# SandAI-org/MagiAttention

Measured on AMD Instinct MI355X. Metric: attention TFLOPS/sec fwd+bwd (whole-job; per-GPU = value/n_gpus); cp scaling at seqlen 64k, higher is better.
Workload: dtype bf16; 1 GPU; dense_causal_64k_h32_d128; seqlen=65536, heads=32, kv_heads=32, head_dim=128, mask=causal, global_batch=1, parallelism=cp1

## Files before the change

### magi_attention/csrc/ffa_bwd.hip

```cpp

#include <hip/hip_runtime.h>
#include <math.h>
#include <stdlib.h>

#include "../../include/magi_ffa.h"
#include "ffa_device.h"

#define BWD_BN 32
#define BWD_BM 32

DEV_INLINE bool wave_alive(int m0, int qe) { return m0 < qe; }

struct BwdParams {
  const bf16_t* dout;
  const bf16_t* q;
  const bf16_t* k;
  const bf16_t* v;
  const void* out;
  const float* lse;
  float* dq;
  float* dk;
  float* dv;
  float* dpsum;
  const int* q_ranges;
  const int* k_ranges;
  const int* attn_type_map;
  int hq, hk, gqa;
  float scale;
  float softcap;
  long long total_q, total_k;
  int head_major;
  int work_nx, work_ny, work_nz;
  int head_mult;
  int head_off;
  int n_heads_launch;
  const int* seg_starts;
};

template <bool OUT_F32>
__global__ __launch_bounds__(256) void bwd_preprocess_kernel(BwdParams p, int d,
                                                             long long n_rows) {
  const long long row = (long long)blockIdx.x * 4 + (threadIdx.x >> 6);
  if (row >= n_rows) return;
  const int lane = threadIdx.x & 63;
  const int per = d / 64;
  const bf16_t* do_p = p.dout + row * d;
  float acc = 0.f;
  for (int e = 0; e < per; ++e) {
    const int idx = lane * per + e;
    const float dov = (float)do_p[idx];
    float ov;
    if (OUT_F32)
      ov = ((const float*)p.out)[row * d + idx];
    else
      ov = (float)((const bf16_t*)p.out)[row * d + idx];
    acc += dov * ov;
  }
#pragma unroll
  for (int s = 32; s > 0; s >>= 1) acc += __shfl_xor(acc, s, 64);
  if (lane == 0) p.dpsum[row] = acc;
}


template <int D, bool HAS_SOFTCAP, int MODE, int WAVES>
__global__ __launch_bounds__(64 * WAVES, WAVES == 8 ? 2 : 1)
void ffa_bwd_dkv_kernel(BwdParams p) {
  static_assert(WAVES == 4 || (WAVES == 8 && D != 192), "unsupported shape");
  constexpr int NBUF = (MODE != 0 && WAVES == 8) ? 3 : 2;
  constexpr bool WANT_DV = MODE != 2;
  constexpr bool WANT_DK = MODE != 1;
  constexpr bool V_IN_LDS = MODE == 0;
  constexpr int DF = D / 16;
  constexpr int DT = D / 32;
  constexpr int ROWB = (D == 192) ? 512 : D * 2;
  constexpr int ROWE = ROWB / 2;
  constexpr int VSLOTS = D / 8;
  constexpr int SW32M = ROWB / 32 - 1;
  auto swz = [](int row, int byte_off) {
    return byte_off ^ ((row & SW32M) << 5);
  };
  const long long work_total =
      (long long)p.work_nx * p.work_ny * p.work_nz;
  const long long grid_span = (long long)gridDim.x * gridDim.y * gridDim.z;
  const long long w_first = blockIdx.x +
      (long long)gridDim.x * (blockIdx.y + (long long)gridDim.y * blockIdx.z);
  for (long long w = w_first; w < work_total; w += grid_span) {
  const int wx = (int)(w % p.work_nx);
  const long long w2 = w / p.work_nx;
  const int wy = (int)(w2 % p.work_ny);
  const int wz = (int)(w2 / p.work_ny);
  const int ri = wz;
  const int hidx = p.head_major ? wx : wy;
  const int h = p.head_off + hidx * p.head_mult;
  const int wb = p.head_major ? wy : wx;
  const int ks = p.k_ranges[2 * ri], ke = p.k_ranges[2 * ri + 1];
  const int nblk0 = ks + wb * (BWD_BN * WAVES);
  if (nblk0 >= ke) continue;
  const int seg0 = p.seg_starts ? p.seg_starts[ri] : ri;
  const int seg1 = p.seg_starts ? p.seg_starts[ri + 1] : ri + 1;
  int qs, qe, atype;

  const int tid = threadIdx.x;
  const int lane = tid & 63;
  const int wave = tid >> 6;
  if (WAVES == 8 && wave >= 4) asm volatile("s_setprio 1");

  const int lo32 = lane & 31;
  const int hi = lane >> 5;

  const int n0 = nblk0 + wave * BWD_BN;
  const bool wave_live = n0 < ke;

  const float sl2 = HAS_SOFTCAP ? p.softcap * 1.4426950408889634f
                                : p.scale * 1.4426950408889634f;
  const float cap_pre = HAS_SOFTCAP ? p.scale / p.softcap : 0.f;
  const float log2e = 1.4426950408889634f;

  const int kh = h / p.gqa;
  const size_t k_pitch = (size_t)p.hk * D;
  const size_t q_pitch = (size_t)p.hq * D;

  constexpr int QITER =
      (V_IN_LDS && D == 128 && WAVES == 8) ? BWD_BM : 2 * BWD_BM;
  constexpr int NSUB = QITER / BWD_BM;
  constexpr int KVLDS = V_IN_LDS ? 2 * WAVES * BWD_BN * ROWB : 0;
  constexpr int LSELDS = V_IN_LDS ? 0 : NBUF * 2 * QITER * 4;
  static_assert(NBUF * 2 * QITER * ROWB + LSELDS + KVLDS <= 163840,
                "LDS budget");
  __shared__ __attribute__((aligned(16))) char smem[
      NBUF * 2 * QITER * ROWB + LSELDS + KVLDS];
  auto lds_q = [&](int buf) -> __bf16* {
    return (__bf16*)(smem + (2 * buf) * QITER * ROWB);
  };
  auto lds_do = [&](int buf) -> __bf16* {
    return (__bf16*)(smem + (2 * buf + 1) * QITER * ROWB);
  };
  auto lds_lse = [&](int buf) -> float* {
    return (float*)(smem + NBUF * 2 * QITER * ROWB + buf * 2 * QITER * 4);
  };
  __bf16* lds_kt = (__bf16*)(smem + NBUF * 2 * QITER * ROWB + LSELDS) +
                   wave * BWD_BN * ROWE;
  __bf16* lds_vt = (__bf16*)(smem + NBUF * 2 * QITER * ROWB + LSELDS +
                             KVLDS / 2) +
                   wave * BWD_BN * ROWE;

  const int krow = n0 + lo32;
  const int kcl = min(krow, ke - 1);
  const bf16_t* kp_row = p.k + (size_t)kcl * k_pitch + (size_t)kh * D + hi * 8;
  bf16x8 kfA[V_IN_LDS ? 1 : DF], vfA[(WANT_DK && !V_IN_LDS) ? DF : 1];
  if constexpr (!V_IN_LDS) {
    const bf16_t* vp = p.v + (size_t)kcl * k_pitch + (size_t)kh * D;
#pragma unroll
    for (int dd = 0; dd < DF; ++dd) {
      kfA[dd] = *(const bf16x8*)(kp_row - hi * 8 + dd * 16 + hi * 8);
      if constexpr (WANT_DK)
        vfA[dd] = *(const bf16x8*)(vp + dd * 16 + hi * 8);
    }
  }
  constexpr int ROWS_PER_GLDS_V = 1024 / ROWB;
  if constexpr (V_IN_LDS) {
#pragma unroll
    for (int gi = 0; gi < BWD_BN / ROWS_PER_GLDS_V; ++gi) {
      const int r0v = ROWS_PER_GLDS_V * gi;
      const int r = r0v + lane / (ROWB / 16);
      const int c = lane % (ROWB / 16);
      const int kr = min(n0 + r, ke - 1);
      int cs = c ^ ((r & SW32M) << 1);
      if (cs >= VSLOTS) cs = 0;
      const int csw = cs * 8;
      __builtin_amdgcn_global_load_lds(
          (const __attribute__((address_space(1))) unsigned int*)(
              p.k + (size_t)kr * k_pitch + (size_t)kh * D + csw),
          (__attribute__((address_space(3))) unsigned int*)&lds_kt[r0v * ROWE],
          16, 0, 0);
      __builtin_amdgcn_global_load_lds(
          (const __attribute__((address_space(1))) unsigned int*)(
              p.v + (size_t)kr * k_pitch + (size_t)kh * D + csw),
          (__attribute__((address_space(3))) unsigned int*)&lds_vt[r0v * ROWE],
          16, 0, 0);
    }
  }

  const int nlast = min(nblk0 + BWD_BN * WAVES, ke) - 1;
  int q_lo = 0, q_hi = 0, wq_lo = 0, wq_hi = 0;
  auto seg_bounds = [&]() {
    q_lo = qs; q_hi = qe;
    if (atype == 1 || atype == 3) q_lo = max(q_lo, nblk0 - (ke - qe));
    if (atype == 2 || atype == 3) q_hi = min(q_hi, nlast - (ks - qs) + 1);
    wq_lo = qs; wq_hi = qe;
    if (atype == 1 || atype == 3) wq_lo = max(wq_lo, n0 - (ke - qe));
    if (atype == 2 || atype == 3)
      wq_hi = min(wq_hi, (n0 + BWD_BN - 1) - (ks - qs) + 1);
  };

  f32x16 acc_dk[WANT_DK ? DT : 1], acc_dv[WANT_DV ? DT : 1];
#pragma unroll
  for (int dt = 0; dt < DT; ++dt) {
    if constexpr (WANT_DK) acc_dk[dt] = (f32x16)(0.f);
    if constexpr (WANT_DV) acc_dv[dt] = (f32x16)(0.f);
  }

  constexpr int ROWS_PER_GLDS = 1024 / ROWB;
  constexpr int GLDS_TOTAL = QITER / ROWS_PER_GLDS;
  static_assert(NBUF == 2 || GLDS_TOTAL % WAVES == 0, "uniform stage count");
  constexpr int GLDS_PER_WAVE =
      (GLDS_TOTAL % WAVES == 0) ? GLDS_TOTAL / WAVES : 0;
  auto stage_glds = [&](int buf, int m0x) {
#pragma unroll
    for (int gi0 = 0; gi0 < (GLDS_TOTAL + WAVES - 1) / WAVES; ++gi0) {
      const int gi = gi0 * WAVES + wave;
      if (GLDS_TOTAL % WAVES != 0 && gi >= GLDS_TOTAL) break;
      const int r0 = ROWS_PER_GLDS * gi;
      const int r = r0 + lane / (ROWB / 16);
      const int c = lane % (ROWB / 16);
      const int qrow = min(m0x + r, qe - 1);
      int cs = c ^ ((r & SW32M) << 1);
      if (cs >= VSLOTS) cs = 0;
      const int csw = cs * 8;
      __builtin_amdgcn_global_load_lds(
          (const __attribute__((address_space(1))) unsigned int*)(
              p.q + (size_t)qrow * q_pitch + (size_t)h * D + csw),
          (__attribute__((address_space(3))) unsigned int*)&lds_q(buf)[r0 * ROWE],
          16, 0, 0);
      __builtin_amdgcn_global_load_lds(
          (const __attribute__((address_space(1))) unsigned int*)(
              p.dout + (size_t)qrow * q_pitch + (size_t)h * D + csw),
          (__attribute__((address_space(3))) unsigned int*)&lds_do(buf)[r0 * ROWE],
          16, 0, 0);
    }
    if constexpr (!V_IN_LDS) {
#pragma unroll
      for (int sg = 0; sg < NSUB; ++sg) {
        const int qr = min(m0x + sg * BWD_BM + lo32, qe - 1);
        const float* src = (lane < 32) ? p.lse + (size_t)qr * p.hq + h
                                       : p.dpsum + (size_t)qr * p.hq + h;
        __builtin_amdgcn_global_load_lds(
            (const __attribute__((address_space(1))) unsigned int*)src,
            (__attribute__((address_space(3))) unsigned int*)(
                lds_lse(buf) + sg * 2 * BWD_BM),
            4, 0, 0);
      }
    }
  };

  constexpr int GOPS = 2 * GLDS_PER_WAVE + 2;
  int cur = 0;
  for (int seg = seg0; seg < seg1; ++seg) {
  qs = p.q_ranges[2 * seg];
  qe = p.q_ranges[2 * seg + 1];
  atype = p.attn_type_map ? p.attn_type_map[seg] : 0;
  if (qe <= qs) continue;
  seg_bounds();
  if (q_lo >= q_hi) continue;
  cur = 0;
  stage_glds(0, q_lo);
  if constexpr (NBUF == 3) stage_glds(1, q_lo + QITER);

  for (int m0 = q_lo; m0 < q_hi; m0 += QITER) {
    pipe_barrier<NBUF == 3 ? GOPS : 0>();
    if constexpr (NBUF == 3) {
      stage_glds(cur == 0 ? 2 : cur - 1, m0 + 2 * QITER);
    } else {
      if (m0 + QITER < q_hi) stage_glds(cur ^ 1, m0 + QITER);
    }
#pragma unroll
    for (int sub = 0; sub < NSUB; ++sub) {
    const int ms = m0 + sub * BWD_BM;
    if (ms >= q_hi) break;
    const __bf16* lqb = lds_q(cur) + sub * BWD_BM * ROWE;
    const __bf16* ldb = lds_do(cur) + sub * BWD_BM * ROWE;
    const float* lse_t = nullptr;
    const float* dps_t = nullptr;
    float lsedp_reg = 0.f;
    if constexpr (!V_IN_LDS) {
      lse_t = lds_lse(cur) + sub * 2 * BWD_BM;
      dps_t = lse_t + BWD_BM;
    } else {
      const int qr = min(ms + lo32, qe - 1);
      lsedp_reg = (lane < 32) ? p.lse[(size_t)qr * p.hq + h]
                              : p.dpsum[(size_t)qr * p.hq + h];
    }
    auto lse_at = [&](int rl) -> float {
      if constexpr (!V_IN_LDS) return lse_t[rl];
      return __uint_as_float(__builtin_amdgcn_ds_bpermute(
          rl << 2, __float_as_uint(lsedp_reg)));
    };
    auto dps_at = [&](int rl) -> float {
      if constexpr (!V_IN_LDS) return dps_t[rl];
      return __uint_as_float(__builtin_amdgcn_ds_bpermute(
          (32 + rl) << 2, __float_as_uint(lsedp_reg)));
    };

    if (wave_live && ms + BWD_BM > wq_lo && ms < wq_hi) {
      f32x16 s = (f32x16)(0.f), dp = (f32x16)(0.f);
      if constexpr (V_IN_LDS) {
        const char* kt_c = (const char*)lds_kt;
        const char* vt_c = (const char*)lds_vt;
#pragma unroll
        for (int dd = 0; dd < DF; ++dd) {
          const int off = swz(lo32, lo32 * ROWB + dd * 32 + hi * 16);
          bf16x8 dof = *(const bf16x8*)((const char*)ldb + off);
          bf16x8 vf = *(const bf16x8*)(vt_c + off);
          dp = __builtin_amdgcn_mfma_f32_32x32x16_bf16(dof, vf, dp, 0, 0, 0);
          bf16x8 qf = *(const bf16x8*)((const char*)lqb + off);
          bf16x8 kf = *(const bf16x8*)(kt_c + off);
          s = __builtin_amdgcn_mfma_f32_32x32x16_bf16(qf, kf, s, 0, 0, 0);
        }
      } else {
#pragma unroll
      for (int dd = 0; dd < DF; ++dd) {
        const int off = swz(lo32, lo32 * ROWB + dd * 32 + hi * 16);
        bf16x8 qf = *(const bf16x8*)((const char*)lqb + off);
        s = __builtin_amdgcn_mfma_f32_32x32x16_bf16(qf, kfA[dd], s, 0, 0, 0);
        if constexpr (WANT_DK) {
          bf16x8 dof = *(const bf16x8*)((const char*)ldb + off);
          dp = __builtin_amdgcn_mfma_f32_32x32x16_bf16(dof, vfA[dd], dp, 0, 0, 0);
        }
      }
      }

      const int kk = n0 + lo32;
      float* pv = (float*)&s;
      float* dsv = (float*)&dp;
      const bool interior =
          (ms + BWD_BM <= wq_hi) && (ms >= qs) && (n0 + BWD_BN <= ke) &&
          !((atype == 1 || atype == 3) && (n0 + BWD_BN - 1 > ms + (ke - qe))) &&
          !((atype == 2 || atype == 3) && (n0 < ms + BWD_BM - 1 + (ks - qs)));
      bool all_live = interior;
      if (interior) {
#pragma unroll
        for (int r = 0; r < 16; ++r) {
          const float lq = lse_at(crow(r, hi));
          all_live = all_live && (lq != INFINITY) && (lq != -INFINITY);
        }
      }
      if (__all(all_live) && !HAS_SOFTCAP) {
#pragma unroll
        for (int r = 0; r < 16; ++r) {
          const int rl = crow(r, hi);
          const float pij = fast_exp2(s[r] * sl2 - lse_at(rl) * log2e);
          if constexpr (WANT_DV) pv[r] = pij;
          if constexpr (WANT_DK)
            dsv[r] = pij * (dp[r] - dps_at(rl)) * p.scale;
        }
      } else {
#pragma unroll
        for (int r = 0; r < 16; ++r) {
          const int qrow = ms + crow(r, hi);
          const float lq = (qrow < qe) ? lse_at(crow(r, hi)) : INFINITY;
          bool ok = (qrow < wq_hi) && (qrow >= qs) && lq != INFINITY &&
                    lq != -INFINITY && kk < ke;
          if (atype == 1 || atype == 3) ok = ok && (kk - qrow <= ke - qe);
          if (atype == 2 || atype == 3) ok = ok && (kk - qrow >= ks - qs);
          float sv = s[r];
          float dscale = p.scale;
          float t;
          if (HAS_SOFTCAP) {
            const float th = tanhf(sv * cap_pre);
            t = th * sl2;
            dscale = p.scale * (1.f - th * th);
          } else {
            t = sv * sl2;
          }
          const float pij = ok ? fast_exp2(t - lq * log2e) : 0.f;
          if constexpr (WANT_DV) pv[r] = pij;
          if constexpr (WANT_DK)
            dsv[r] = pij * (dp[r] - dps_at(crow(r, hi))) * dscale;
        }
      }

      {
        const int qhalf = (lane >> 4) & 1;
        const int jrow = (lane & 15) >> 2;
        const int row0 = 8 * hi + jrow;
        const int row1 = 8 * hi + 4 + jrow;
        const int q_base = (int)(unsigned long long)(
            (__attribute__((address_space(3))) const char*)lqb);
        const int do_base = (int)(unsigned long long)(
            (__attribute__((address_space(3))) const char*)ldb);
        const int lane8 = (lane & 3) * 8;
        const int sw0 = (row0 & SW32M) << 5;
        const int sw1 = (row1 & SW32M) << 5;
        const int rb0 = row0 * ROWB + lane8;
        const int rb1 = row1 * ROWB + lane8;
        const int sw2 = ((row0 + 16) & SW32M) << 5;
        const int sw3 = ((row1 + 16) & SW32M) << 5;
        const int rb2 = (row0 + 16) * ROWB + lane8;
        const int rb3 = (row1 + 16) * ROWB + lane8;
        auto pipe_mm = [&](int tbase, bf16x8 a0, bf16x8 a1, f32x16* acc) {
          bf16x8 bcur = tr16_frag(tbase + rb0 + ((16 * qhalf * 2) ^ sw0),
                                  tbase + rb1 + ((16 * qhalf * 2) ^ sw1));
#pragma unroll
          for (int j = 0; j < 2 * DT; ++j) {
            bf16x8 bnext = bcur;
            if (j + 1 < 2 * DT) {
              const int dcoln = (((j + 1) >> 1) * 32 + 16 * qhalf) * 2;
              if ((j + 1) & 1)
                bnext = tr16_frag(tbase + rb2 + (dcoln ^ sw2),
                                  tbase + rb3 + (dcoln ^ sw3));
              else
                bnext = tr16_frag(tbase + rb0 + (dcoln ^ sw0),
                                  tbase + rb1 + (dcoln ^ sw1));
            }
            acc[j >> 1] = __builtin_amdgcn_mfma_f32_32x32x16_bf16(
                (j & 1) ? a1 : a0, bcur, acc[j >> 1], 0, 0, 0);
            bcur = bnext;
          }
        };
        if constexpr (MODE == 1) {
          pipe_mm(do_base, cframe_to_afrag(pv, 0), cframe_to_afrag(pv, 1),
                  acc_dv);
        } else if constexpr (MODE == 2) {
          pipe_mm(q_base, cframe_to_afrag(dsv, 0), cframe_to_afrag(dsv, 1),
                  acc_dk);
        } else {
          bf16x8 pa0 = cframe_to_afrag(pv, 0);
          bf16x8 pa1 = cframe_to_afrag(pv, 1);
          bf16x8 da0 = cframe_to_afrag(dsv, 0);
          bf16x8 da1 = cframe_to_afrag(dsv, 1);
#pragma unroll
          for (int dt = 0; dt < DT; ++dt) {
            const int dcol = (dt * 32 + 16 * qhalf) * 2;
            bf16x8 bdo = tr16_frag(do_base + rb0 + (dcol ^ sw0),
                                   do_base + rb1 + (dcol ^ sw1));
            acc_dv[dt] = __builtin_amdgcn_mfma_f32_32x32x16_bf16(
                pa0, bdo, acc_dv[dt], 0, 0, 0);
            bf16x8 bq = tr16_frag(q_base + rb0 + (dcol ^ sw0),
                                  q_base + rb1 + (dcol ^ sw1));
            acc_dk[dt] = __builtin_amdgcn_mfma_f32_32x32x16_bf16(
                da0, bq, acc_dk[dt], 0, 0, 0);
            bf16x8 bdo1 = tr16_frag(do_base + rb2 + (dcol ^ sw2),
                                    do_base + rb3 + (dcol ^ sw3));
            acc_dv[dt] = __builtin_amdgcn_mfma_f32_32x32x16_bf16(
                pa1, bdo1, acc_dv[dt], 0, 0, 0);
            bf16x8 bq1 = tr16_frag(q_base + rb2 + (dcol ^ sw2),
                                   q_base + rb3 + (dcol ^ sw3));
            acc_dk[dt] = __builtin_amdgcn_mfma_f32_32x32x16_bf16(
                da1, bq1, acc_dk[dt], 0, 0, 0);
          }
        }
      }
    }
    }
    cur = (NBUF == 3) ? (cur == 2 ? 0 : cur + 1) : (cur ^ 1);
  }
  __syncthreads();
  }

  if (wave_live) {
#pragma unroll
  for (int r = 0; r < 16; ++r) {
    const int kr = n0 + crow(r, hi);
    if (kr >= ke) continue;
    float* dkp = p.dk + (size_t)kr * k_pitch + (size_t)kh * D;
    float* dvp = p.dv + (size_t)kr * k_pitch + (size_t)kh * D;
#pragma unroll
    for (int dt = 0; dt < DT; ++dt) {
      if constexpr (WANT_DK) {
        if (acc_dk[dt][r] != 0.f)
          unsafeAtomicAdd(dkp + dt * 32 + lo32, acc_dk[dt][r]);
      }
      if constexpr (WANT_DV) {
        if (acc_dv[dt][r] != 0.f)
          unsafeAtomicAdd(dvp + dt * 32 + lo32, acc_dv[dt][r]);
      }
    }
  }
  }
  if constexpr (MODE == 0) break;
  }
}


template <int D, bool HAS_SOFTCAP, int WAVES>
__global__ __launch_bounds__(64 * WAVES, WAVES == 8 ? 1 : 2)
void ffa_bwd_dq_kernel(BwdParams p) {
  static_assert(WAVES == 4 || (WAVES == 8 && D != 192), "unsupported shape");
  constexpr int NBUF = WAVES == 8 ? 3 : 2;
  constexpr int DF = D / 16;
  constexpr int DT = D / 32;
  constexpr int ROWB = (D == 192) ? 512 : D * 2;
  constexpr int ROWE = ROWB / 2;
  constexpr int VSLOTS = D / 8;
  constexpr int SW32M = ROWB / 32 - 1;
  auto swz = [](int row, int byte_off) {
    return byte_off ^ ((row & SW32M) << 5);
  };
  const long long work_total =
      (long long)p.work_nx * p.work_ny * p.work_nz;
  const long long grid_span = (long long)gridDim.x * gridDim.y * gridDim.z;
  for (long long w = blockIdx.x +
           (long long)gridDim.x * (blockIdx.y + (long long)gridDim.y * blockIdx.z);
       w < work_total; w += grid_span) {
  const int wx = (int)(w % p.work_nx);
  const long long w2 = w / p.work_nx;
  const int wy = (int)(w2 % p.work_ny);
  const int wz = (int)(w2 / p.work_ny);
  const int ri = wz;
  const int h = p.head_major ? wx : wy;
  const int wb = p.head_major ? wy : wx;
  const int qs = p.q_ranges[2 * ri], qe = p.q_ranges[2 * ri + 1];
  const int mblk0 = qs + wb * (BWD_BM * WAVES);
  if (mblk0 >= qe) continue;
  const int seg0 = p.seg_starts ? p.seg_starts[ri] : ri;
  const int seg1 = p.seg_starts ? p.seg_starts[ri + 1] : ri + 1;
  int ks, ke, atype;

  const int tid = threadIdx.x;
  const int lane = tid & 63;
  const int wave = tid >> 6;
  if (WAVES == 8 && wave >= 4) asm volatile("s_setprio 1");

  const int lo32 = lane & 31;
  const int hi = lane >> 5;

  const int m0 = mblk0 + wave * BWD_BM;
  const int qrow = m0 + lo32;
  const bool qvalid = qrow < qe && m0 < qe;
  const int qcl = qvalid ? qrow : (qe - 1);

  const float sl2 = HAS_SOFTCAP ? p.softcap * 1.4426950408889634f
                                : p.scale * 1.4426950408889634f;
  const float cap_pre = HAS_SOFTCAP ? p.scale / p.softcap : 0.f;
  const float log2e = 1.4426950408889634f;

  const int kh = h / p.gqa;
  const size_t k_pitch = (size_t)p.hk * D;
  const size_t q_pitch = (size_t)p.hq * D;

  constexpr int KITER = 2 * BWD_BN;
  static_assert(NBUF * 2 * KITER * ROWB <= 163840, "LDS budget");
  __shared__ __attribute__((aligned(16))) char smem[NBUF * 2 * KITER * ROWB];
  auto lds_k = [&](int buf) -> __bf16* {
    return (__bf16*)(smem + (2 * buf) * KITER * ROWB);
  };
  auto lds_v = [&](int buf) -> __bf16* {
    return (__bf16*)(smem + (2 * buf + 1) * KITER * ROWB);
  };

  bf16x8 qf[DF], dof[DF];
  {
    const bf16_t* qp = p.q + (size_t)qcl * q_pitch + (size_t)h * D;
    const bf16_t* dp = p.dout + (size_t)qcl * q_pitch + (size_t)h * D;
#pragma unroll
    for (int dd = 0; dd < DF; ++dd) {
      qf[dd] = *(const bf16x8*)(qp + dd * 16 + hi * 8);
      dof[dd] = *(const bf16x8*)(dp + dd * 16 + hi * 8);
    }
  }
  const float lse_q = qvalid ? p.lse[(size_t)qrow * p.hq + h] : INFINITY;
  const float dpsum_q = qvalid ? p.dpsum[(size_t)qrow * p.hq + h] : 0.f;
  const bool row_live = qvalid && lse_q != INFINITY && lse_q != -INFINITY;

  const int mlast = min(mblk0 + BWD_BM * WAVES, qe) - 1;
  int k_lo = 0, k_hi = 0, wk_lo = 0, wk_hi = 0;
  auto seg_bounds = [&]() {
    k_lo = ks; k_hi = ke;
    if (atype == 1 || atype == 3) k_hi = min(k_hi, mlast + (ke - qe) + 1);
    if (atype == 2 || atype == 3) k_lo = max(k_lo, mblk0 + (ks - qs));
    wk_lo = ks; wk_hi = ke;
    if (atype == 1 || atype == 3)
      wk_hi = min(wk_hi, min(m0 + BWD_BM, qe) - 1 + (ke - qe) + 1);
    if (atype == 2 || atype == 3) wk_lo = max(wk_lo, m0 + (ks - qs));
  };

  f32x16 acc_dq[DT];
#pragma unroll
  for (int dt = 0; dt < DT; ++dt) acc_dq[dt] = (f32x16)(0.f);

  constexpr int ROWS_PER_GLDS = 1024 / ROWB;
  static_assert(KITER / WAVES >= ROWS_PER_GLDS, "stage rows per wave");
  constexpr int GLDS_PER_WAVE = (KITER / WAVES) / ROWS_PER_GLDS;
  auto stage_glds = [&](int buf, int n0x) {
#pragma unroll
    for (int gi = 0; gi < GLDS_PER_WAVE; ++gi) {
      const int r0 = (KITER / WAVES) * wave + ROWS_PER_GLDS * gi;
      const int r = r0 + lane / (ROWB / 16);
      const int c = lane % (ROWB / 16);
      const int kr = min(n0x + r, ke - 1);
      int cs = c ^ ((r & SW32M) << 1);
      if (cs >= VSLOTS) cs = 0;
      const int csw = cs * 8;
      __builtin_amdgcn_global_load_lds(
          (const __attribute__((address_space(1))) unsigned int*)(
              p.k + (size_t)kr * k_pitch + (size_t)kh * D + csw),
          (__attribute__((address_space(3))) unsigned int*)&lds_k(buf)[r0 * ROWE],
          16, 0, 0);
      __builtin_amdgcn_global_load_lds(
          (const __attribute__((address_space(1))) unsigned int*)(
              p.v + (size_t)kr * k_pitch + (size_t)kh * D + csw),
          (__attribute__((address_space(3))) unsigned int*)&lds_v(buf)[r0 * ROWE],
          16, 0, 0);
    }
  };

  constexpr int GOPS = 2 * GLDS_PER_WAVE;
  int cur = 0;
  for (int seg = seg0; seg < seg1; ++seg) {
  ks = p.k_ranges[2 * seg];
  ke = p.k_ranges[2 * seg + 1];
  atype = p.attn_type_map ? p.attn_type_map[seg] : 0;
  if (ke <= ks) continue;
  seg_bounds();
  if (k_lo >= k_hi) continue;
  cur = 0;
  stage_glds(0, k_lo);
  if constexpr (NBUF == 3) stage_glds(1, k_lo + KITER);

  for (int n0 = k_lo; n0 < k_hi; n0 += KITER) {
    pipe_barrier<NBUF == 3 ? GOPS : 0>();
    if constexpr (NBUF == 3) {
      stage_glds(cur == 0 ? 2 : cur - 1, n0 + 2 * KITER);
    } else {
      if (n0 + KITER < k_hi) stage_glds(cur ^ 1, n0 + KITER);
    }
#pragma unroll
    for (int sub = 0; sub < 2; ++sub) {
    const int ns = n0 + sub * BWD_BN;
    if (ns >= k_hi) break;
    const __bf16* lkb = lds_k(cur) + sub * BWD_BN * ROWE;
    const __bf16* lvb = lds_v(cur) + sub * BWD_BN * ROWE;

    if (wave_alive(m0, qe) && ns + BWD_BN > wk_lo && ns < wk_hi) {
      f32x16 sA = (f32x16)(0.f), dpA = (f32x16)(0.f);
#pragma unroll
      for (int dd = 0; dd < DF; ++dd) {
        const int off = swz(lo32, lo32 * ROWB + dd * 32 + hi * 16);
        bf16x8 kf = *(const bf16x8*)((const char*)lkb + off);
        bf16x8 vf = *(const bf16x8*)((const char*)lvb + off);
        sA = __builtin_amdgcn_mfma_f32_32x32x16_bf16(kf, qf[dd], sA, 0, 0, 0);
        dpA = __builtin_amdgcn_mfma_f32_32x32x16_bf16(vf, dof[dd], dpA, 0, 0, 0);
      }

      float dsv[16];
      const bool interior =
          (qrow < qe) && row_live && (ns >= ks) && (ns + BWD_BN <= ke) &&
          !((atype == 1 || atype == 3) && (ns + BWD_BN - 1 > m0 + (ke - qe))) &&
          !((atype == 2 || atype == 3) && (ns < m0 + 31 + (ks - qs)));
      if (__all(interior) && !HAS_SOFTCAP) {
        const float lsc = lse_q * log2e;
#pragma unroll
        for (int r = 0; r < 16; ++r) {
          const float pij = fast_exp2(sA[r] * sl2 - lsc);
          dsv[r] = pij * (dpA[r] - dpsum_q) * p.scale;
        }
      } else {
#pragma unroll
        for (int r = 0; r < 16; ++r) {
          const int kk = ns + crow(r, hi);
          bool ok = row_live && kk < ke && kk >= ks;
          if (atype == 1 || atype == 3) ok = ok && (kk - qrow <= ke - qe);
          if (atype == 2 || atype == 3) ok = ok && (kk - qrow >= ks - qs);
          float sv = sA[r];
          float dscale = p.scale;
          float t;
          if (HAS_SOFTCAP) {
            const float th = tanhf(sv * cap_pre);
            t = th * sl2;
            dscale = p.scale * (1.f - th * th);
          } else {
            t = sv * sl2;
          }
          const float pij = ok ? fast_exp2(t - lse_q * log2e) : 0.f;
          dsv[r] = pij * (dpA[r] - dpsum_q) * dscale;
        }
      }

      bf16x8 dsa0 = cframe_to_afrag(dsv, 0);
      bf16x8 dsa1 = cframe_to_afrag(dsv, 1);
      {
        const int qhalf2 = (lane >> 4) & 1;
        const int jrow = (lane & 15) >> 2;
        const int row0 = 8 * hi + jrow;
        const int row1 = 8 * hi + 4 + jrow;
        const int k_base = (int)(unsigned long long)(
            (__attribute__((address_space(3))) const char*)lkb);
        const int lane8 = (lane & 3) * 8;
        const int sw0 = (row0 & SW32M) << 5;
        const int sw1 = (row1 & SW32M) << 5;
        const int rb0 = row0 * ROWB + lane8;
        const int rb1 = row1 * ROWB + lane8;
        const int sw2 = ((row0 + 16) & SW32M) << 5;
        const int sw3 = ((row1 + 16) & SW32M) << 5;
        const int rb2 = (row0 + 16) * ROWB + lane8;
        const int rb3 = (row1 + 16) * ROWB + lane8;
        bf16x8 bcur = tr16_frag(k_base + rb0 + ((16 * qhalf2 * 2) ^ sw0),
                                k_base + rb1 + ((16 * qhalf2 * 2) ^ sw1));
#pragma unroll
        for (int j = 0; j < 2 * DT; ++j) {
          bf16x8 bnext = bcur;
          if (j + 1 < 2 * DT) {
            const int dcoln = (((j + 1) >> 1) * 32 + 16 * qhalf2) * 2;
            if ((j + 1) & 1)
              bnext = tr16_frag(k_base + rb2 + (dcoln ^ sw2),
                                k_base + rb3 + (dcoln ^ sw3));
            else
              bnext = tr16_frag(k_base + rb0 + (dcoln ^ sw0),
                                k_base + rb1 + (dcoln ^ sw1));
          }
          acc_dq[j >> 1] = __builtin_amdgcn_mfma_f32_32x32x16_bf16(
              (j & 1) ? dsa1 : dsa0, bcur, acc_dq[j >> 1], 0, 0, 0);
          bcur = bnext;
        }
      }
    }
    }
    cur = (NBUF == 3) ? (cur == 2 ? 0 : cur + 1) : (cur ^ 1);
  }
  __syncthreads();
  }

#pragma unroll
  for (int r = 0; r < 16; ++r) {
    const int qr = m0 + crow(r, hi);
    if (qr >= qe) continue;
    float* dst = p.dq + (size_t)qr * q_pitch + (size_t)h * D;
#pragma unroll
    for (int dt = 0; dt < DT; ++dt) {
      const float val = acc_dq[dt][r];
      if (val != 0.f) unsafeAtomicAdd(dst + dt * 32 + lo32, val);
    }
  }
  }
}


extern "C" int magi_ffa_bwd_preprocess(const magi_ffa_bwd_args* a) {
  if (!a || !a->dout || !a->out || !a->dpsum) return -1;
  BwdParams p{};
  p.dout = (const bf16_t*)a->dout;
  p.out = a->out;
  p.dpsum = a->dpsum;
  const long long n_rows = a->total_q * a->hq;
  if (n_rows == 0) return 0;
  dim3 grid((unsigned)((n_rows + 3) / 4)), block(256);
  hipStream_t s = (hipStream_t)a->stream;
  if (a->out_is_fp32)
    hipLaunchKernelGGL((bwd_preprocess_kernel<true>), grid, block, 0, s, p,
                       a->d, n_rows);
  else
    hipLaunchKernelGGL((bwd_preprocess_kernel<false>), grid, block, 0, s, p,
                       a->d, n_rows);
  return (int)hipGetLastError();
}

static int fill_bwd_params(const magi_ffa_bwd_args* a, BwdParams* p) {
  if (!a || !a->dout || !a->q || !a->k || !a->v || !a->lse) return -1;
  if (a->d != 64 && a->d != 128 && a->d != 192) return -2;
  if (a->hq % a->hk != 0) return -3;
  if (a->n_ranges <= 0) return 1;
  p->dout = (const bf16_t*)a->dout;
  p->q = (const bf16_t*)a->q;
  p->k = (const bf16_t*)a->k;
  p->v = (const bf16_t*)a->v;
  p->out = a->out;
  p->lse = a->lse;
  p->dq = a->dq;
  p->dk = a->dk;
  p->dv = a->dv;
  p->dpsum = a->dpsum;
  p->q_ranges = a->q_ranges;
  p->k_ranges = a->k_ranges;
  p->attn_type_map = a->attn_type_map;
  p->hq = a->hq;
  p->hk = a->hk;
  p->gqa = a->hq / a->hk;
  p->scale = a->softmax_scale;
  p->softcap = a->softcap;
  p->total_q = a->total_q;
  p->total_k = a->total_k;
  p->seg_starts = a->seg_starts;
  p->head_mult = 1;
  p->head_off = 0;
  p->n_heads_launch = a->hq;
  if (a->cu_margin & 0xFFFF0000) {
    p->head_mult = (a->cu_margin >> 24) & 0xFF;
    p->head_off = (a->cu_margin >> 16) & 0xFF;
    p->n_heads_launch = a->hq / p->head_mult;
  }
  return 0;
}

static int env_int(const char* name, int dflt) {
  const char* e = getenv(name);
  return e ? atoi(e) : dflt;
}

static dim3 cap_grid(dim3 grid, int margin, int wg_per_cu) {
  if (margin <= 0) return grid;
  const long long total = (long long)grid.x * grid.y * grid.z;
  long long cap = (long long)(256 - margin) * wg_per_cu;
  if (cap < 1) cap = 1;
  if (cap > total) cap = total;
  return dim3((unsigned)cap, 1, 1);
}

struct BwdKnobs {
  int head_major;
  int bigseq;
};

static BwdKnobs dq_knobs(const magi_ffa_bwd_args* a) {
  const int hm = ((long long)a->total_k * a->d * 4 <= (16 << 20)) ? 1 : 0;
  return {env_int("MAGI_BWD_HEAD_MAJOR", hm),
          env_int("MAGI_BWD_DQ_BIGSEQ", 8192)};
}

template <int D>
static void launch_dq(int waves, bool sc, dim3 grid, hipStream_t s,
                      const BwdParams& p) {
#define GO(SC, W)                                                          \
  hipLaunchKernelGGL((ffa_bwd_dq_kernel<D, SC, W>), grid, dim3(64 * W), 0, \
                     s, p)
  if constexpr (D != 192) {
    if (waves == 8) {
      if (sc) GO(true, 8); else GO(false, 8);
      return;
    }
  }
  if (sc) GO(true, 4); else GO(false, 4);
#undef GO
}

extern "C" int magi_ffa_bwd_dq(const magi_ffa_bwd_args* a) {
  BwdParams p;
  int rc = fill_bwd_params(a, &p);
  if (rc) return rc > 0 ? 0 : rc;
  const BwdKnobs knobs = dq_knobs(a);
  p.head_major = knobs.head_major;
  const int W = (a->d != 192 && a->max_seqlen_k >= knobs.bigseq) ? 8 : 4;
  if (a->n_ranges > 65535) return -5;
  const int qspan = BWD_BM * W;
  const int qblocks = (int)((a->total_q + qspan - 1) / qspan);
  dim3 grid = p.head_major ? dim3(a->hq, qblocks, (unsigned)a->n_ranges)
                           : dim3(qblocks, a->hq, (unsigned)a->n_ranges);
  p.work_nx = grid.x; p.work_ny = grid.y; p.work_nz = grid.z;
  grid = cap_grid(grid, a->cu_margin & 0xFFFF, W == 4 ? 2 : 1);
  hipStream_t s = (hipStream_t)a->stream;
  const bool sc = a->softcap > 0.f;
  if (a->d == 64) launch_dq<64>(W, sc, grid, s, p);
  else if (a->d == 192) launch_dq<192>(W, sc, grid, s, p);
  else launch_dq<128>(W, sc, grid, s, p);
  return (int)hipGetLastError();
}

static BwdKnobs dkv_knobs() {
  return {env_int("MAGI_BWD_HEAD_MAJOR", 1), env_int("MAGI_BWD_BIGSEQ", 1024)};
}

template <int D, int MODE>
static void launch_dkv(int waves, bool sc, dim3 grid, hipStream_t s,
                       const BwdParams& p) {
#define GO(SC, W)                                                        \
  hipLaunchKernelGGL((ffa_bwd_dkv_kernel<D, SC, MODE, W>), grid,         \
                     dim3(64 * W), 0, s, p)
  if constexpr (D != 192) {
    if (waves == 8) {
      if (sc) GO(true, 8); else GO(false, 8);
      return;
    }
  }
  if (sc) GO(true, 4); else GO(false, 4);
#undef GO
}

template <int MODE>
static int launch_bwd_dkv(const magi_ffa_bwd_args* a) {
  BwdParams p;
  int rc = fill_bwd_params(a, &p);
  if (rc) return rc > 0 ? 0 : rc;
  const BwdKnobs knobs = dkv_knobs();
  p.head_major = knobs.head_major;
  const int W = (a->d != 192 && a->max_seqlen_k >= knobs.bigseq) ? 8 : 4;
  const int span = BWD_BN * W;
  const int nblocks = (a->max_seqlen_k + span - 1) / span;
  if (a->n_ranges > 65535) return -5;
  dim3 grid = p.head_major
                  ? dim3(p.n_heads_launch, nblocks, (unsigned)a->n_ranges)
                  : dim3(nblocks, p.n_heads_launch, (unsigned)a->n_ranges);
  p.work_nx = grid.x; p.work_ny = grid.y; p.work_nz = grid.z;
  if constexpr (MODE != 0)
    grid = cap_grid(grid, a->cu_margin & 0xFFFF, W == 4 ? 2 : 1);
  hipStream_t s = (hipStream_t)a->stream;
  const bool sc = a->softcap > 0.f;
  if (a->d == 64) launch_dkv<64, MODE>(W, sc, grid, s, p);
  else if (a->d == 192) {
    if constexpr (MODE != 0) launch_dkv<192, MODE>(W, sc, grid, s, p);
    else return -6;
  } else launch_dkv<128, MODE>(W, sc, grid, s, p);
  return (int)hipGetLastError();
}

extern "C" int magi_ffa_bwd_dkv(const magi_ffa_bwd_args* a) {
  return launch_bwd_dkv<0>(a);
}

extern "C" int magi_ffa_bwd_dv(const magi_ffa_bwd_args* a) {
  return launch_bwd_dkv<1>(a);
}

extern "C" int magi_ffa_bwd_dk(const magi_ffa_bwd_args* a) {
  return launch_bwd_dkv<2>(a);
}

extern "C" int magi_ffa_bwd(const magi_ffa_bwd_args* a) {
  int rc = magi_ffa_bwd_dq(a);
  if (rc) return rc;
  return magi_ffa_bwd_dkv(a);
}
```

Before: 601.3 TFLOPS/s.

## Prefetch LSE/dpsum across iterations, use raw LDS loads, reverse causal block order

In the V-in-LDS backward path, LSE and dpsum values for the next Q tile are now loaded into registers one iteration ahead, so per-sub-tile global loads leave the critical path. LSE values are gathered once into an array and reused. Q/dO staging goes through inline-asm global_load_lds instructions that the compiler does not track for waits. The dQ-side kernel also reverses the Q-block order for causal masks so the heaviest blocks are scheduled first, reducing the tail. Untracked loads depend on the existing barriers for correctness, and the extra registers may raise pressure.

```diff
diff --git a/magi_attention/csrc/ffa_bwd.hip b/magi_attention/csrc/ffa_bwd.hip
--- a/magi_attention/csrc/ffa_bwd.hip
+++ b/magi_attention/csrc/ffa_bwd.hip
@@ -10,6 +10,12 @@
 #define BWD_BM 32
 
 DEV_INLINE bool wave_alive(int m0, int qe) { return m0 < qe; }
+
+DEV_INLINE void glds16_untracked(const void* gsrc, int lds_byte) {
+  const int m0v = __builtin_amdgcn_readfirstlane(lds_byte);
+  asm volatile("s_mov_b32 m0, %0\n\ts_nop 0\n\tglobal_load_lds_dwordx4 %1, off"
+               :: "s"(m0v), "v"(gsrc) : "memory", "m0");
+}
 
 struct BwdParams {
   const bf16_t* dout;
@@ -205,6 +211,10 @@
   static_assert(NBUF == 2 || GLDS_TOTAL % WAVES == 0, "uniform stage count");
   constexpr int GLDS_PER_WAVE =
       (GLDS_TOTAL % WAVES == 0) ? GLDS_TOTAL / WAVES : 0;
+  const bf16_t* q_head = p.q + (size_t)h * D;
+  const bf16_t* do_head = p.dout + (size_t)h * D;
+  const int smem_byte = (int)(unsigned long long)(
+      (__attribute__((address_space(3))) const char*)smem);
   auto stage_glds = [&](int buf, int m0x) {
 #pragma unroll
     for (int gi0 = 0; gi0 < (GLDS_TOTAL + WAVES - 1) / WAVES; ++gi0) {
@@ -217,14 +227,20 @@
       int cs = c ^ ((r & SW32M) << 1);
       if (cs >= VSLOTS) cs = 0;
       const int csw = cs * 8;
+      const size_t eoff = (size_t)qrow * q_pitch + (unsigned)csw;
+      if constexpr (V_IN_LDS) {
+        const int lq = smem_byte + (2 * buf * QITER + r0) * ROWB;
+        glds16_untracked(q_head + eoff, lq);
+        glds16_untracked(do_head + eoff, lq + QITER * ROWB);
+        continue;
+      }
       __builtin_amdgcn_global_load_lds(
-          (const __attribute__((address_space(1))) unsigned int*)(
-              p.q + (size_t)qrow * q_pitch + (size_t)h * D + csw),
+          (const __attribute__((address_space(1))) unsigned int*)(q_head + eoff),
           (__attribute__((address_space(3))) unsigned int*)&lds_q(buf)[r0 * ROWE],
           16, 0, 0);
       __builtin_amdgcn_global_load_lds(
           (const __attribute__((address_space(1))) unsigned int*)(
-              p.dout + (size_t)qrow * q_pitch + (size_t)h * D + csw),
+              do_head + eoff),
           (__attribute__((address_space(3))) unsigned int*)&lds_do(buf)[r0 * ROWE],
           16, 0, 0);
     }
@@ -244,6 +260,16 @@
   };
 
   constexpr int GOPS = 2 * GLDS_PER_WAVE + 2;
+  float lse_nxt[V_IN_LDS ? NSUB : 1] = {}, dps_nxt[V_IN_LDS ? NSUB : 1] = {};
+  auto load_lsedp = [&](int m0x) {
+#pragma unroll
+    for (int sg = 0; sg < NSUB; ++sg) {
+      const int qr = min(m0x + sg * BWD_BM + lo32, qe - 1);
+      const size_t roff = (size_t)qr * p.hq + h;
+      lse_nxt[sg] = p.lse[roff];
+      dps_nxt[sg] = p.dpsum[roff];
+    }
+  };
   int cur = 0;
   for (int seg = seg0; seg < seg1; ++seg) {
   qs = p.q_ranges[2 * seg];
@@ -253,15 +279,28 @@
   seg_bounds();
   if (q_lo >= q_hi) continue;
   cur = 0;
+  if constexpr (V_IN_LDS) load_lsedp(q_lo);
   stage_glds(0, q_lo);
   if constexpr (NBUF == 3) stage_glds(1, q_lo + QITER);
 
   for (int m0 = q_lo; m0 < q_hi; m0 += QITER) {
     pipe_barrier<NBUF == 3 ? GOPS : 0>();
+    float lse_cur[V_IN_LDS ? NSUB : 1] = {}, dps_cur[V_IN_LDS ? NSUB : 1] = {};
+    if constexpr (V_IN_LDS) {
+#pragma unroll
+      for (int sg = 0; sg < NSUB; ++sg) {
+        lse_cur[sg] = lse_nxt[sg];
+        dps_cur[sg] = dps_nxt[sg];
+        asm volatile("" : "+v"(lse_cur[sg]), "+v"(dps_cur[sg]));
+      }
+    }
     if constexpr (NBUF == 3) {
       stage_glds(cur == 0 ? 2 : cur - 1, m0 + 2 * QITER);
     } else {
-      if (m0 + QITER < q_hi) stage_glds(cur ^ 1, m0 + QITER);
+      if (m0 + QITER < q_hi) {
+        if constexpr (V_IN_LDS) load_lsedp(m0 + QITER);
+        stage_glds(cur ^ 1, m0 + QITER);
+      }
     }
 #pragma unroll
     for (int sub = 0; sub < NSUB; ++sub) {
@@ -271,24 +310,21 @@
     const __bf16* ldb = lds_do(cur) + sub * BWD_BM * ROWE;
     const float* lse_t = nullptr;
     const float* dps_t = nullptr;
-    float lsedp_reg = 0.f;
+    const float lse_reg = lse_cur[V_IN_LDS ? sub : 0];
+    const float dps_reg = dps_cur[V_IN_LDS ? sub : 0];
     if constexpr (!V_IN_LDS) {
       lse_t = lds_lse(cur) + sub * 2 * BWD_BM;
       dps_t = lse_t + BWD_BM;
-    } else {
-      const int qr = min(ms + lo32, qe - 1);
-      lsedp_reg = (lane < 32) ? p.lse[(size_t)qr * p.hq + h]
-                              : p.dpsum[(size_t)qr * p.hq + h];
     }
     auto lse_at = [&](int rl) -> float {
       if constexpr (!V_IN_LDS) return lse_t[rl];
       return __uint_as_float(__builtin_amdgcn_ds_bpermute(
-          rl << 2, __float_as_uint(lsedp_reg)));
+          rl << 2, __float_as_uint(lse_reg)));
     };
     auto dps_at = [&](int rl) -> float {
       if constexpr (!V_IN_LDS) return dps_t[rl];
       return __uint_as_float(__builtin_amdgcn_ds_bpermute(
-          (32 + rl) << 2, __float_as_uint(lsedp_reg)));
+          rl << 2, __float_as_uint(dps_reg)));
     };
 
     if (wave_live && ms + BWD_BM > wq_lo && ms < wq_hi) {
@@ -326,11 +362,14 @@
           (ms + BWD_BM <= wq_hi) && (ms >= qs) && (n0 + BWD_BN <= ke) &&
           !((atype == 1 || atype == 3) && (n0 + BWD_BN - 1 > ms + (ke - qe))) &&
           !((atype == 2 || atype == 3) && (n0 < ms + BWD_BM - 1 + (ks - qs)));
+      float lqv[16];
+#pragma unroll
+      for (int r = 0; r < 16; ++r) lqv[r] = lse_at(crow(r, hi));
       bool all_live = interior;
       if (interior) {
 #pragma unroll
         for (int r = 0; r < 16; ++r) {
-          const float lq = lse_at(crow(r, hi));
+          const float lq = lqv[r];
           all_live = all_live && (lq != INFINITY) && (lq != -INFINITY);
         }
       }
@@ -338,7 +377,7 @@
 #pragma unroll
         for (int r = 0; r < 16; ++r) {
           const int rl = crow(r, hi);
-          const float pij = fast_exp2(s[r] * sl2 - lse_at(rl) * log2e);
+          const float pij = fast_exp2(s[r] * sl2 - lqv[r] * log2e);
           if constexpr (WANT_DV) pv[r] = pij;
           if constexpr (WANT_DK)
             dsv[r] = pij * (dp[r] - dps_at(rl)) * p.scale;
@@ -347,7 +386,7 @@
 #pragma unroll
         for (int r = 0; r < 16; ++r) {
           const int qrow = ms + crow(r, hi);
-          const float lq = (qrow < qe) ? lse_at(crow(r, hi)) : INFINITY;
+          const float lq = (qrow < qe) ? lqv[r] : INFINITY;
           bool ok = (qrow < wq_hi) && (qrow >= qs) && lq != INFINITY &&
                     lq != -INFINITY && kk < ke;
           if (atype == 1 || atype == 3) ok = ok && (kk - qrow <= ke - qe);
@@ -498,12 +537,15 @@
   const int wz = (int)(w2 / p.work_ny);
   const int ri = wz;
   const int h = p.head_major ? wx : wy;
-  const int wb = p.head_major ? wy : wx;
+  const int wb_lin = p.head_major ? wy : wx;
   const int qs = p.q_ranges[2 * ri], qe = p.q_ranges[2 * ri + 1];
-  const int mblk0 = qs + wb * (BWD_BM * WAVES);
-  if (mblk0 >= qe) continue;
+  const int nqb = (qe - qs + BWD_BM * WAVES - 1) / (BWD_BM * WAVES);
+  if (wb_lin >= nqb) continue;
   const int seg0 = p.seg_starts ? p.seg_starts[ri] : ri;
   const int seg1 = p.seg_starts ? p.seg_starts[ri + 1] : ri + 1;
+  const int at0 = p.attn_type_map ? p.attn_type_map[seg0] : 0;
+  const int wb = (at0 == 1 || at0 == 3) ? nqb - 1 - wb_lin : wb_lin;
+  const int mblk0 = qs + wb * (BWD_BM * WAVES);
   int ks, ke, atype;
 
   const int tid = threadIdx.x;
```

Measured after the change: 607.7 TFLOPS/s (median of 6 runs). 1.1% higher.
